# sun2ot/DiffMM

Hardware: NVIDIA B200
Metric: denoise_topk_rebuild_users_per_sec (higher is better)
Workload: dtype bf16

## Files before the change

diffmm_b200/csrc/adj.cu:

```cuda
#include "common.cuh"

#include <cub/device/device_radix_sort.cuh>

namespace {

__global__ void __launch_bounds__(256) expand_users_kernel(const int64_t* __restrict__ row_ptr, int64_t n_users,
                                                           int32_t* __restrict__ edge_user,
                                                           const int32_t* __restrict__ items, int64_t n_items,
                                                           int32_t* __restrict__ status) {
  const int64_t u = ((int64_t)blockIdx.x * blockDim.x + threadIdx.x) >> 5;
  const int lane = threadIdx.x & 31;
  if (u >= n_users) return;
  const int64_t b = row_ptr[u], e = row_ptr[u + 1];
  for (int64_t j = b + lane; j < e; j += 32) {
    edge_user[j] = (int32_t)u;
    const int32_t it = items[j];
    if ((it < 0 || it >= n_items) && status) atomicOr(status, 2);
  }
}

__device__ __forceinline__ int64_t lower_bound_item(const int32_t* __restrict__ items_sorted, int64_t n_edges, int64_t it) {
  int64_t lo = 0, hi = n_edges;
  while (lo < hi) {
    const int64_t mid = (lo + hi) >> 1;
    if ((int64_t)__ldg(items_sorted + mid) < it) lo = mid + 1; else hi = mid;
  }
  return lo;
}
__global__ void __launch_bounds__(256) offsets_dinv_kernel(const int64_t* __restrict__ row_ptr,
                                                           const int32_t* __restrict__ items_sorted, int64_t n_users,
                                                           int64_t n_items, int64_t n_edges, int64_t* __restrict__ item_ptr,
                                                           double* __restrict__ dinv) {
  __shared__ int64_t lb[256];
  const int64_t user_blocks = (n_users + 255) / 256;
  if ((int64_t)blockIdx.x < user_blocks) {
    const int64_t u = (int64_t)blockIdx.x * 256 + threadIdx.x;
    if (u < n_users) dinv[u] = 1.0 / sqrt((double)(row_ptr[u + 1] - row_ptr[u] + 1));
    return;
  }
  const int64_t it = ((int64_t)blockIdx.x - user_blocks) * 255 + threadIdx.x;
  lb[threadIdx.x] = it < n_items ? lower_bound_item(items_sorted, n_edges, it) : n_edges;
  __syncthreads();
  if (threadIdx.x == 255 || it >= n_items) return;
  const int64_t b = lb[threadIdx.x], e = lb[threadIdx.x + 1];
  item_ptr[it] = b;
  if (it + 1 == n_items) item_ptr[n_items] = n_edges;
  dinv[n_users + it] = 1.0 / sqrt((double)(e - b + 1));
}

__global__ void __launch_bounds__(256) fill_adj_kernel(const int64_t* __restrict__ row_ptr,
                                                       const int32_t* __restrict__ items,
                                                       const int32_t* __restrict__ edge_user,
                                                       const int64_t* __restrict__ item_ptr,
                                                       const int32_t* __restrict__ items_sorted,
                                                       const int32_t* __restrict__ users_by_item,
                                                       const double* __restrict__ dinv, int64_t n_users,
                                                       int64_t n_items, int64_t n_edges, int64_t* __restrict__ adj_ptr,
                                                       int32_t* __restrict__ adj_idx, float* __restrict__ adj_val) {
  const int64_t j = (int64_t)blockIdx.x * blockDim.x + threadIdx.x;
  const int64_t N = n_users + n_items;
  if (j < n_edges) {
    {
      const int64_t u = edge_user[j];
      const int32_t it = items[j];
      const int64_t o = j + u + 1;
      adj_idx[o] = (int32_t)(n_users + it);
      adj_val[o] = (float)((dinv[u] * 1.0) * dinv[n_users + it]);
    }
    {
      const int64_t it = items_sorted[j];
      const int32_t u = users_by_item[j];
      const int64_t o = n_edges + n_users + j + it;
      adj_idx[o] = u;
      adj_val[o] = (float)((dinv[n_users + it] * 1.0) * dinv[u]);
    }
  }
  if (j < N) {
    const double d = dinv[j];
    int64_t start, self;
    if (j < n_users) {
      start = row_ptr[j] + j;
      self = start;
    } else {
      const int64_t it = j - n_users;
      start = n_edges + n_users + item_ptr[it] + it;
      self = n_edges + n_users + item_ptr[it + 1] + it;
    }
    adj_ptr[j] = start;
    adj_idx[self] = (int32_t)j;
    adj_val[self] = (float)((d * 1.0) * d);
    if (j == N - 1) adj_ptr[N] = 2 * n_edges + N;
  }
}

struct Workspace {
  int32_t* edge_user;
  int32_t* items_sorted;
  int32_t* users_by_item;
  int32_t* item_count;
  int64_t* item_ptr;
  double* dinv;
  void* cub_tmp;
  size_t cub_bytes;
};

inline size_t align256(size_t x) { return (x + 255) & ~(size_t)255; }

inline size_t carve(Workspace& w, void* base, int64_t U, int64_t I, int64_t E) {
  uint8_t* p = (uint8_t*)base;
  size_t off = 0;
  const size_t e4 = align256((size_t)(E > 0 ? E : 1) * 4);
  w.edge_user = (int32_t*)(p + off); off += e4;
  w.items_sorted = (int32_t*)(p + off); off += e4;
  w.users_by_item = (int32_t*)(p + off); off += e4;
  w.item_count = (int32_t*)(p + off); off += align256((size_t)(I + 1) * 4);
  w.item_ptr = (int64_t*)(p + off); off += align256((size_t)(I + 1) * 8);
  w.dinv = (double*)(p + off); off += align256((size_t)(U + I) * 8);
  w.cub_tmp = p + off;
  return off;
}

}

extern "C" int64_t dmm_build_adj_workspace_bytes(int64_t n_users, int64_t n_items, int64_t n_edges) {
  Workspace w;
  const size_t fixed = carve(w, nullptr, n_users, n_items, n_edges);
  return (int64_t)(fixed + (size_t)(32u << 20) + (size_t)(n_edges > 0 ? n_edges : 0));
}

extern "C" int dmm_build_norm_adj_csr(dmm_ctx* ctx, const int64_t* row_ptr, const int32_t* items, int64_t n_users,
                                      int64_t n_items, int64_t n_edges, int64_t* adj_ptr, int32_t* adj_idx,
                                      float* adj_val, void* workspace, int64_t workspace_bytes, int32_t* status,
                                      void* stream) {
  DMM_CHECK_ARG(ctx && row_ptr && adj_ptr && adj_idx && adj_val && workspace, "dmm_build_norm_adj_csr: null argument");
  DMM_CHECK_ARG(n_users > 0 && n_items > 0 && n_edges >= 0, "dmm_build_norm_adj_csr: bad sizes");
  DMM_CHECK_ARG(n_users + n_items < (1LL << 31) && n_edges < (1LL << 31), "dmm_build_norm_adj_csr: int32 index overflow");
  DMM_CHECK_ARG(n_edges == 0 || items, "dmm_build_norm_adj_csr: null items");
  cudaStream_t st = (cudaStream_t)stream;
  Workspace w;
  const size_t fixed = carve(w, workspace, n_users, n_items, n_edges);
  DMM_CHECK_ARG((size_t)workspace_bytes > fixed, "dmm_build_norm_adj_csr: workspace too small");
  w.cub_bytes = (size_t)workspace_bytes - fixed;

  expand_users_kernel<<<(unsigned)dmm_ceil_div(n_users * 32, 256), 256, 0, st>>>(row_ptr, n_users, w.edge_user, items, n_items,
                                                                                status);
  DMM_LAUNCH_CHECK();
  if (n_edges > 0) {
    int end_bit = 1;
    while ((1LL << end_bit) < n_items) ++end_bit;
    size_t need = 0;
    DMM_CUDA(cub::DeviceRadixSort::SortPairs(nullptr, need, items, w.items_sorted, w.edge_user, w.users_by_item,
                                             (int)n_edges, 0, end_bit, st));
    if (need > w.cub_bytes) {
      dmm_set_error("dmm_build_norm_adj_csr: sort scratch needs %zu bytes, %zu available", need, w.cub_bytes);
      return DMM_ERR_WORKSPACE;
    }
    DMM_CUDA(cub::DeviceRadixSort::SortPairs(w.cub_tmp, need, items, w.items_sorted, w.edge_user, w.users_by_item,
                                             (int)n_edges, 0, end_bit, st));
  }
  const int64_t N = n_users + n_items;
  offsets_dinv_kernel<<<(unsigned)(dmm_ceil_div(n_users, 256) + dmm_ceil_div(n_items, 255)), 256, 0, st>>>(
      row_ptr, w.items_sorted, n_users, n_items, n_edges, w.item_ptr, w.dinv);
  DMM_LAUNCH_CHECK();
  const int64_t work = n_edges > N ? n_edges : N;
  fill_adj_kernel<<<(unsigned)dmm_ceil_div(work, 256), 256, 0, st>>>(row_ptr, items, w.edge_user, w.item_ptr, w.items_sorted,
                                                                    w.users_by_item, w.dinv, n_users, n_items, n_edges,
                                                                    adj_ptr, adj_idx, adj_val);
  DMM_LAUNCH_CHECK();
  return DMM_OK;
}
```

diffmm_b200/csrc/topk.cu:

```cuda
#include "common.cuh"

#include <stdlib.h>

namespace {

constexpr int TOPK_NB_LOG2 = 11;
constexpr int TOPK_NB = 1 << TOPK_NB_LOG2;
constexpr int TOPK_CAND = 1024;
constexpr int TOPK_V4 = 8;
constexpr int TOPK_SEG_COLS = 8192;
constexpr int TOPK_MERGE_CAP = 2048;

struct SegCfg {
  int mode;
  int S;
  int seg_cols;
  int last_len;
};
__device__ __forceinline__ bool seg_eligible(const SegCfg& sg, int k) {
  return k > 0 && k <= 256 && k <= sg.last_len && (int64_t)sg.S * k <= TOPK_MERGE_CAP;
}

__device__ __forceinline__ float fmax_nan(float a, float b) {
  float r;
// ... 403 lines not shown
      const float xs[4] = {v[j].x, v[j].y, v[j].z, v[j].w};
#pragma unroll
      for (int e = 0; e < 4; ++e) push(open && !(xs[e] < Lf), xs[e], 4 * (tid + NT * j) + e);
    }
  }
  if (n_cols & 3) push(has_tail && !(tail_v < Lf), tail_v, tail_col);
  __syncthreads();
  const int m = sm.ncand;
  constexpr int RANK_MAX = 512;
  if (m > RANK_MAX || m < k) {
    __syncthreads();
    topk_row_generic<NT, false>(sm, nullptr, row, n_cols, k, o0, user, out_users, out_items, col_off);
    return;
  }
  for (int c = tid; c < m; c += NT) {
    const uint32_t my_key = sm.cand[c];
    const int my_col = sm.cand_col[c];
    int before = 0;
    if (m > k) {
      for (int j = 0; j < m; ++j) {
        const uint32_t kj = sm.cand[j];
        const int cj = sm.cand_col[j];
        before += (kj > my_key || (kj == my_key && cj < my_col)) ? 1 : 0;
      }
    }
    sm.bucket[c] = before < k ? my_col : 0x7FFFFFFF;
  }
  __syncthreads();
  for (int c = tid; c < m; c += NT) {
    const int my_col = sm.bucket[c];
    if (my_col == 0x7FFFFFFF) continue;
    int pos = 0;
    for (int j = 0; j < m; ++j) pos += (sm.bucket[j] < my_col) ? 1 : 0;
    out_items[o0 + pos] = my_col + col_off;
    if (out_users) out_users[o0 + pos] = user;
  }
}

__global__ void __launch_bounds__(128) topk_merge_kernel(const float* __restrict__ scores, int64_t ld, int64_t n_rows,
                                                         const int64_t* __restrict__ out_ptr, int64_t row_base,
                                                         int32_t* __restrict__ out_users, int32_t* __restrict__ out_items,
                                                         const int32_t* __restrict__ order, SegCfg sg,
                                                         const int32_t* __restrict__ seg_tmp, const int32_t* __restrict__ live) {
  __shared__ uint32_t key[TOPK_MERGE_CAP];
  __shared__ int col[TOPK_MERGE_CAP];
  __shared__ int sel[TOPK_MERGE_CAP];
  if ((int64_t)blockIdx.x >= n_rows) return;
  if (live && (int64_t)blockIdx.x >= (int64_t)*live) return;
  const int64_t r = order ? (int64_t)order[blockIdx.x] : (int64_t)blockIdx.x;
  const int64_t o0 = out_ptr[r];
  const int k = (int)(out_ptr[r + 1] - o0);
  if (!seg_eligible(sg, k)) return;
  const int m = sg.S * k;
  const int32_t* list = seg_tmp + (int64_t)sg.S * (o0 - out_ptr[0]);
  const float* row = scores + r * ld;
  for (int c = threadIdx.x; c < m; c += 128) {
    const int cc = list[c];
    col[c] = cc;
    key[c] = order_key(__ldg(row + cc));
  }
  __syncthreads();
  for (int c = threadIdx.x; c < m; c += 128) {
    const uint32_t my_key = key[c];
    const int my_col = col[c];
    int before = 0;
    for (int j = 0; j < m; ++j) before += (key[j] > my_key || (key[j] == my_key && col[j] < my_col)) ? 1 : 0;
    sel[c] = before < k ? my_col : 0x7FFFFFFF;
  }
  __syncthreads();
  const int32_t user = (int32_t)(row_base + r);
  for (int c = threadIdx.x; c < m; c += 128) {
    const int my_col = sel[c];
    if (my_col == 0x7FFFFFFF) continue;
    int pos = 0;
    for (int j = 0; j < m; ++j) pos += (sel[j] < my_col) ? 1 : 0;
    out_items[o0 + pos] = my_col;
    if (out_users) out_users[o0 + pos] = user;
  }
}

template <int NT>
void launch_reg(const float* scores, int64_t ld, int64_t n_rows, int n_cols, const int64_t* out_ptr, int64_t row_base,
                int32_t* out_users, int32_t* out_items, int32_t* status, const int32_t* order, SegCfg sg, int32_t* seg_tmp,
                const int32_t* live, cudaStream_t st) {
  const int64_t blocks = sg.mode == 1 ? n_rows * sg.S : n_rows;
  topk_rows_reg_kernel<NT><<<(unsigned)blocks, NT, 0, st>>>(scores, ld, n_rows, n_cols, out_ptr, row_base, out_users,
                                                           out_items, status, order, sg, seg_tmp, live);
}

constexpr int PRUNE_KMAX = 64;
constexpr int PRUNE_RATIO = 4;
constexpr int PRUNE_CAND = 512;

struct PruneArgs {
  const float* scores;
  int64_t ld;
  const float* cmax;
  int64_t ld_cmax;
  int n_chunks, n_cols;
  int64_t n_rows;
  const int64_t* out_ptr;
  int64_t row_base;
  int32_t* out_users;
  int32_t* out_items;
  int32_t* status;
  const int32_t* order;
  int32_t* left_count;
  int32_t* left_rows;
};

__host__ __device__ __forceinline__ int prune_kmax(int n_chunks) {
  const int nw = n_chunks <= 64 * 4 * TOPK_V4 ? 2 : (n_chunks <= 256 * 4 * TOPK_V4 ? 8 : 16);
  return PRUNE_KMAX < 32 * nw ? PRUNE_KMAX : 32 * nw;
}
__host__ __device__ __forceinline__ bool prune_k_ok(int64_t k, int n_chunks, int64_t n_cols) {
  return k <= prune_kmax(n_chunks) && k * PRUNE_RATIO <= n_chunks && k <= n_cols;
}

struct alignas(16) PruneSmem {
  uint32_t key[PRUNE_CAND];
  int col[PRUNE_CAND];
  int sel[PRUNE_CAND];
  uint32_t red[32];
  int ncand, nsel, ncand2;
  uint32_t lk;
};

__device__ __forceinline__ float key_to_float(uint32_t L) {
  return (L == 0u) ? __uint_as_float(0xFF800000u) : __uint_as_float((L & 0x80000000u) ? (L ^ 0x80000000u) : ~L);
}

template <int NT>
__global__ void __launch_bounds__(NT) topk_pruned_kernel(const PruneArgs a) {
  __shared__ PruneSmem sm;
  constexpr int NW = NT / 32;
  if ((int64_t)blockIdx.x >= a.n_rows) return;
  const int64_t r = a.order ? (int64_t)a.order[blockIdx.x] : (int64_t)blockIdx.x;
  const int tid = threadIdx.x, lane = tid & 31, wid = tid >> 5;
  const int n_chunks = a.n_chunks;

  const float* crow = a.cmax + r * a.ld_cmax;
  const int n4 = n_chunks >> 2;
  const float4* crow4 = reinterpret_cast<const float4*>(crow);
  float4 v[TOPK_V4];
#pragma unroll
  for (int j = 0; j < TOPK_V4; ++j) {
    v[j] = make_float4(0.f, 0.f, 0.f, 0.f);
    if (tid + NT * j < n4) v[j] = __ldg(crow4 + tid + NT * j);
  }
  const int tail_col = (n4 << 2) + tid;
  const bool has_tail = tid < (n_chunks & 3);
  float tail_v = 0.f;
  if (has_tail) tail_v = __ldg(crow + tail_col);

  const int64_t o0 = a.out_ptr[r];
  const int k = (int)(a.out_ptr[r + 1] - o0);
  if (k <= 0) return;
  auto defer = [&]() {
    if (tid == 0) a.left_rows[atomicAdd(a.left_count, 1)] = (int32_t)r;
  };
  if (!prune_k_ok(k, n_chunks, a.n_cols)) {
    defer();
    return;
  }
  const float NEG_INF = __uint_as_float(0xFF800000u);
  const int jfull = n4 / NT, jrem = n4 - jfull * NT;
  float pmax[TOPK_V4];
  float tmaxf = has_tail ? fmax_nan(tail_v, NEG_INF) : NEG_INF;
#pragma unroll
  for (int j = 0; j < TOPK_V4; ++j) {
    pmax[j] = NEG_INF;
    if (j < jfull || (j == jfull && tid < jrem)) {
      pmax[j] = fmax_nan(fmax_nan(v[j].x, v[j].y), fmax_nan(v[j].z, v[j].w));
      tmaxf = fmax_nan(tmaxf, pmax[j]);
    }
  }
  const uint32_t tmax = (tmaxf == NEG_INF) ? 0u : order_key(tmaxf);

  const int q = (k + NW - 1) / NW;
  uint32_t wq;
  {
    uint32_t sv = tmax;
#pragma unroll
    for (int k2 = 2; k2 <= 32; k2 <<= 1) {
#pragma unroll
      for (int j = k2 >> 1; j > 0; j >>= 1) {
        const uint32_t other = __shfl_xor_sync(0xffffffffu, sv, j);
        const bool desc = (lane & k2) == 0;
        const bool lower = (lane & j) == 0;
        sv = (lower == desc) ? max(sv, other) : min(sv, other);
      }
    }
    wq = __shfl_sync(0xffffffffu, sv, q - 1);
  }
  if (lane == 0) sm.red[wid] = wq;
  if (tid == 0) {
    sm.ncand = 0;
    sm.nsel = 0;
    sm.ncand2 = 0;
    sm.lk = 0xFFFFFFFFu;
  }
  if (__syncthreads_or(tmaxf != tmaxf)) {
    defer();
    return;
  }
  uint32_t L = 0xFFFFFFFFu;
#pragma unroll
  for (int i = 0; i < NW; ++i) L = min(L, sm.red[i]);
  const float Lf = key_to_float(L);

  auto push = [&](int* counter, bool c, float x, int col) {
    const uint32_t bal = __ballot_sync(0xffffffffu, c);
    if (bal) {
      int base = 0;
      if (lane == 0) base = atomicAdd(counter, __popc(bal));
      base = __shfl_sync(0xffffffffu, base, 0);
      const int pos = base + __popc(bal & ((1u << lane) - 1u));
      if (c && pos < PRUNE_CAND) {
        sm.key[pos] = order_key(x);
        sm.col[pos] = col;
      }
    }
  };
#pragma unroll
  for (int j = 0; j < TOPK_V4; ++j) {
    if (j > jfull) break;
    const bool have = j < jfull || tid < jrem;
    const bool open = have && !(pmax[j] < Lf);
    if (__any_sync(0xffffffffu, open)) {
      const float xs[4] = {v[j].x, v[j].y, v[j].z, v[j].w};
#pragma unroll
      for (int e = 0; e < 4; ++e) push(&sm.ncand, open && !(xs[e] < Lf), xs[e], 4 * (tid + NT * j) + e);
    }
  }
  if (n_chunks & 3) push(&sm.ncand, has_tail && !(tail_v < Lf), tail_v, tail_col);
  __syncthreads();
  const int m = sm.ncand;
  if (m > PRUNE_CAND || m < k) {
    defer();
    return;
  }
  for (int c = tid; c < m; c += NT) {
    const uint32_t my_key = sm.key[c];
    const int my_col = sm.col[c];
    int before = 0;
    if (m > k) {
      for (int j = 0; j < m; ++j) {
        const uint32_t kj = sm.key[j];
        const int cj = sm.col[j];
        before += (kj > my_key || (kj == my_key && cj < my_col)) ? 1 : 0;
      }
    }
    if (before < k) {
      sm.sel[atomicAdd(&sm.nsel, 1)] = my_col;
      atomicMin(&sm.lk, my_key);
    }
  }
  __syncthreads();
  const float Lkf = key_to_float(sm.lk);

  const float* row = a.scores + r * a.ld;
  constexpr int GB = 8;
  for (int i0 = wid; i0 < k; i0 += NW * GB) {
    float xs[GB];
    int cols[GB];
#pragma unroll
    for (int t = 0; t < GB; ++t) {
      const int i = i0 + t * NW;
      cols[t] = i < k ? sm.sel[i] * 32 + lane : 0x7FFFFFFF;
      xs[t] = cols[t] < a.n_cols ? __ldg(row + cols[t]) : NEG_INF;
    }
#pragma unroll
    for (int t = 0; t < GB; ++t) {
      if (i0 + t * NW >= k) break;
      push(&sm.ncand2, cols[t] < a.n_cols && !(xs[t] < Lkf), xs[t], cols[t]);
    }
  }
  __syncthreads();
  const int m2 = sm.ncand2;
  if (m2 > PRUNE_CAND || m2 < k) {
    defer();
    return;
  }
  for (int c = tid; c < m2; c += NT) {
    const uint32_t my_key = sm.key[c];
    const int my_col = sm.col[c];
    int before = 0;
    if (m2 > k) {
      for (int j = 0; j < m2; ++j) {
        const uint32_t kj = sm.key[j];
        const int cj = sm.col[j];
        before += (kj > my_key || (kj == my_key && cj < my_col)) ? 1 : 0;
      }
    }
    sm.sel[c] = before < k ? my_col : 0x7FFFFFFF;
  }
  __syncthreads();
  const int32_t user = (int32_t)(a.row_base + r);
  for (int c = tid; c < m2; c += NT) {
    const int my_col = sm.sel[c];
    if (my_col == 0x7FFFFFFF) continue;
    int pos = 0;
    for (int j = 0; j < m2; ++j) pos += (sm.sel[j] < my_col) ? 1 : 0;
    a.out_items[o0 + pos] = my_col;
    if (a.out_users) a.out_users[o0 + pos] = user;
  }
}

__global__ void __launch_bounds__(256) topk_deferred_kernel(const float* __restrict__ scores, int64_t ld, int n_cols,
                                                            const float* __restrict__ cmax, int64_t ld_cmax, int n_chunks,
                                                            const int64_t* __restrict__ out_ptr, int64_t row_base,
                                                            int32_t* __restrict__ out_users, int32_t* __restrict__ out_items,
                                                            int32_t* __restrict__ status, const int32_t* __restrict__ rows,
                                                            const int32_t* __restrict__ live,
                                                            int32_t* __restrict__ chunk_list, int smem_keys) {
  extern __shared__ uint32_t s_keys[];
  __shared__ TopkSmem<256> sm;
  const int tid = threadIdx.x;
  const int n = *live;
  const int64_t e0 = out_ptr[0];
  for (int slot = blockIdx.x; slot < n; slot += gridDim.x) {
    const int64_t r = rows[slot];
    const int64_t o0 = out_ptr[r];
    int k = (int)(out_ptr[r + 1] - o0);
    if (k > n_cols) {
      if (status && tid == 0) atomicOr(status, 1);
      k = n_cols;
    }
    if (k <= 0) continue;
    const float* row = scores + r * ld;
    const float* crow = cmax + r * ld_cmax;
    bool two_level = (int64_t)k * 2 <= n_chunks;
    if (two_level) {
      bool nan = false;
      for (int i = tid; i < n_chunks; i += 256) {
        const float c = __ldg(crow + i);
        nan |= c != c;
      }
      two_level = !__syncthreads_or(nan);
    }
    if (two_level) {
      int32_t* list = chunk_list + (o0 - e0);
      if (n_chunks <= smem_keys) {
        uint32_t kmin = 0xFFFFFFFFu, kmax = 0u;
        for (int i = tid; i < n_chunks; i += 256) {
          const uint32_t q = order_key(__ldg(crow + i));
          s_keys[i] = q;
          kmin = min(kmin, q);
          kmax = max(kmax, q);
        }
        topk_select_emit<256>(sm, [&](int i) -> uint32_t { return s_keys[i]; }, [](int i) -> int { return i; }, n_chunks, k,
                              true, kmin, kmax, 0, 0, nullptr, list);
      } else {
        topk_select_emit<256>(sm, [&](int i) -> uint32_t { return order_key(__ldg(crow + i)); }, [](int i) -> int { return i; },
                              n_chunks, k, false, 0u, 0u, 0, 0, nullptr, list);
      }
      __syncthreads();
      const int nv = k * 32;
      auto vcol = [&](int i) -> int { return list[i >> 5] * 32 + (i & 31); };
      auto vkey = [&](int i) -> uint32_t {
        const int c = vcol(i);
        return c < n_cols ? order_key(__ldg(row + c)) : 0u;
      };
      if (nv <= smem_keys) {
        uint32_t kmin = 0xFFFFFFFFu, kmax = 0u;
#pragma unroll 4
        for (int i = tid; i < nv; i += 256) {
          const uint32_t q = vkey(i);
          s_keys[i] = q;
          kmin = min(kmin, q);
          kmax = max(kmax, q);
        }
        topk_select_emit<256>(sm, [&](int i) -> uint32_t { return s_keys[i]; }, vcol, nv, k, true, kmin, kmax, o0,
                              (int32_t)(row_base + r), out_users, out_items);
      } else {
        topk_select_emit<256>(sm, vkey, vcol, nv, k, false, 0u, 0u, o0, (int32_t)(row_base + r), out_users, out_items);
      }
    } else {
      topk_row_generic<256, false>(sm, nullptr, row, n_cols, k, o0, (int32_t)(row_base + r), out_users, out_items);
    }
    __syncthreads();
  }
}

SegCfg make_seg(int64_t n_cols) {
  SegCfg sg{0, 0, 0, 0};
  if (n_cols > TOPK_SEG_COLS) {
    sg.S = (int)dmm_ceil_div(n_cols, TOPK_SEG_COLS);
    sg.seg_cols = (int)((dmm_ceil_div(n_cols, sg.S) + 3) / 4 * 4);
    sg.last_len = (int)(n_cols - (int64_t)(sg.S - 1) * sg.seg_cols);
    if (sg.last_len <= 0) sg.S = 0;
  }
  return sg;
}

}

extern "C" int64_t dmm_topk_workspace_bytes(int64_t n_cols, int64_t n_edges) {
  const SegCfg sg = make_seg(n_cols);
  return sg.S > 0 ? (int64_t)sg.S * (n_edges > 0 ? n_edges : 0) * (int64_t)sizeof(int32_t) : 0;
}

static int topk_dispatch(dmm_ctx* ctx, const float* scores, int64_t ld, int64_t n_rows, int64_t n_cols,
                         const int64_t* out_ptr, int64_t row_base, int32_t* out_users, int32_t* out_items, int32_t* status,
                         const int32_t* order, const int32_t* live, void* workspace, int64_t workspace_bytes,
                         int64_t n_edges, cudaStream_t st) {
  constexpr int PER_THREAD = 4 * TOPK_V4;
  static const bool force_generic = getenv("DMM_TOPK_GENERIC") != nullptr;
  static const bool seg_ok = []() { const char* e = getenv("DMM_TOPK_SEG"); return !(e && e[0] == '0'); }();

  SegCfg sg = make_seg(n_cols);
  const bool rows_aligned = (reinterpret_cast<uintptr_t>(scores) & 15u) == 0 && ld % 4 == 0;
  const bool segmented = seg_ok && !force_generic && sg.S > 0 && rows_aligned && workspace != nullptr && n_edges >= 0 &&
                         workspace_bytes >= dmm_topk_workspace_bytes(n_cols, n_edges) && n_rows * (int64_t)sg.S < (1LL << 31);
  if (segmented) {
    sg.mode = 1;
    launch_reg<256>(scores, ld, n_rows, (int)n_cols, out_ptr, row_base, nullptr, nullptr, status, order, sg, (int32_t*)workspace,
                    live, st);
    DMM_LAUNCH_CHECK();
    topk_merge_kernel<<<(unsigned)n_rows, 128, 0, st>>>(scores, ld, n_rows, out_ptr, row_base, out_users, out_items, order, sg,
                                                       (const int32_t*)workspace, live);
    DMM_LAUNCH_CHECK();
    sg.mode = 2;
    topk_edges_kernel<false><<<(unsigned)n_rows, 256, 0, st>>>(scores, ld, n_rows, (int)n_cols, out_ptr, row_base, out_users,
                                                              out_items, status, order, sg, live);
    DMM_LAUNCH_CHECK();
    return DMM_OK;
  }
  sg = SegCfg{0, 0, 0, 0};
  if (force_generic) {
  } else if (n_cols <= 256 * PER_THREAD) {
    launch_reg<256>(scores, ld, n_rows, (int)n_cols, out_ptr, row_base, out_users, out_items, status, order, sg, nullptr, live, st);
  } else if (n_cols <= 512 * PER_THREAD) {
    launch_reg<512>(scores, ld, n_rows, (int)n_cols, out_ptr, row_base, out_users, out_items, status, order, sg, nullptr, live, st);
  } else if (n_cols <= 1024 * PER_THREAD) {
    launch_reg<1024>(scores, ld, n_rows, (int)n_cols, out_ptr, row_base, out_users, out_items, status, order, sg, nullptr, live, st);
  }
  if (force_generic || n_cols > 1024 * PER_THREAD) {
    const size_t smem = (size_t)n_cols * sizeof(uint32_t);
    const size_t cap = (size_t)ctx->max_smem_optin > 40960 ? (size_t)ctx->max_smem_optin - 20480 : 0;
    if (smem <= cap) {
      static DmmPerDeviceOnce smem_once;
      if (smem > 24 * 1024 && smem_once.need(ctx)) {
        DMM_CUDA(cudaFuncSetAttribute(topk_edges_kernel<true>, cudaFuncAttributeMaxDynamicSharedMemorySize, (int)cap));
        smem_once.mark(ctx);
      }
      topk_edges_kernel<true><<<(unsigned)n_rows, 256, smem, st>>>(scores, ld, n_rows, (int)n_cols, out_ptr, row_base,
                                                                  out_users, out_items, status, order, sg, live);
    } else {
      topk_edges_kernel<false><<<(unsigned)n_rows, 256, 0, st>>>(scores, ld, n_rows, (int)n_cols, out_ptr, row_base,
                                                                out_users, out_items, status, order, sg, live);
    }
  }
  DMM_LAUNCH_CHECK();
  return DMM_OK;
}

extern "C" int dmm_topk_edges(dmm_ctx* ctx, const float* scores, int64_t ld, int64_t n_rows, int64_t n_cols,
                              const int64_t* out_ptr, int64_t row_base, int32_t* out_users, int32_t* out_items,
                              int32_t* status, const int32_t* order, void* workspace, int64_t workspace_bytes,
                              int64_t n_edges, void* stream) {
  DMM_CHECK_ARG(ctx && scores && out_ptr && out_items, "dmm_topk_edges: null argument");
  DMM_CHECK_ARG(n_cols > 0 && n_cols < (1LL << 31) && ld >= n_cols, "dmm_topk_edges: bad shape n_cols=%lld ld=%lld",
                (long long)n_cols, (long long)ld);
  DMM_CHECK_ARG(n_rows >= 0 && n_rows < (1LL << 31), "dmm_topk_edges: bad n_rows");
  if (n_rows == 0) return DMM_OK;
  return topk_dispatch(ctx, scores, ld, n_rows, n_cols, out_ptr, row_base, out_users, out_items, status, order, nullptr,
                       workspace, workspace_bytes, n_edges, (cudaStream_t)stream);
}

namespace {
inline size_t prune_align(size_t x) { return (x + 255) & ~(size_t)255; }
inline size_t prune_head_bytes(int64_t n_rows) { return 256 + prune_align((size_t)(n_rows > 0 ? n_rows : 1) * sizeof(int32_t)); }
}

extern "C" int64_t dmm_topk_pruned_workspace_bytes(int64_t n_rows, int64_t n_cols, int64_t n_edges) {
  return (int64_t)prune_head_bytes(n_rows) + (int64_t)prune_align((size_t)(n_edges > 0 ? n_edges : 1) * sizeof(int32_t)) +
         dmm_topk_workspace_bytes(n_cols, n_edges);
}

extern "C" int dmm_topk_edges_pruned(dmm_ctx* ctx, const float* scores, int64_t ld, int64_t n_rows, int64_t n_cols,
                                     const float* cmax, int64_t ld_cmax, const int64_t* out_ptr, int64_t row_base,
                                     int32_t* out_users, int32_t* out_items, int32_t* status, const int32_t* order,
                                     void* workspace, int64_t workspace_bytes, int64_t n_edges, void* stream) {
  DMM_CHECK_ARG(ctx && scores && cmax && out_ptr && out_items && workspace, "dmm_topk_edges_pruned: null argument");
  DMM_CHECK_ARG(n_cols > 0 && n_cols < (1LL << 31) && ld >= n_cols, "dmm_topk_edges_pruned: bad shape n_cols=%lld ld=%lld",
                (long long)n_cols, (long long)ld);
  DMM_CHECK_ARG(n_rows >= 0 && n_rows < (1LL << 31) && n_edges >= 0, "dmm_topk_edges_pruned: bad n_rows / n_edges");
  const int64_t n_chunks = dmm_ceil_div(n_cols, 32);
  DMM_CHECK_ARG(ld_cmax >= n_chunks && ld_cmax % 4 == 0 && (reinterpret_cast<uintptr_t>(cmax) & 15u) == 0,
                "dmm_topk_edges_pruned: cmax rows must be 16-byte aligned with ld_cmax %% 4 == 0 and >= ceil(n_cols / 32)");
  DMM_CHECK_ARG(workspace_bytes >= dmm_topk_pruned_workspace_bytes(n_rows, n_cols, n_edges),
                "dmm_topk_edges_pruned: workspace smaller than dmm_topk_pruned_workspace_bytes");
  if (n_rows == 0) return DMM_OK;
  cudaStream_t st = (cudaStream_t)stream;
  const size_t list_bytes = prune_align((size_t)(n_edges > 0 ? n_edges : 1) * sizeof(int32_t));
  int32_t* const chunk_list = (int32_t*)((uint8_t*)workspace + prune_head_bytes(n_rows));
  uint8_t* const seg_ws = (uint8_t*)workspace + prune_head_bytes(n_rows) + list_bytes;
  const int64_t seg_ws_bytes = workspace_bytes - (int64_t)prune_head_bytes(n_rows) - (int64_t)list_bytes;
  static const bool prune_ok = []() { const char* e = getenv("DMM_TOPK_PRUNE"); return !(e && e[0] == '0'); }();
  if (!prune_ok || n_chunks > 512 * 4 * TOPK_V4 || n_chunks < 8)
    return topk_dispatch(ctx, scores, ld, n_rows, n_cols, out_ptr, row_base, out_users, out_items, status, order, nullptr,
                         seg_ws, seg_ws_bytes, n_edges, st);
  int32_t* left_count = (int32_t*)workspace;
  int32_t* left_rows = (int32_t*)((uint8_t*)workspace + 256);
  DMM_CUDA(cudaMemsetAsync(left_count, 0, sizeof(int32_t), st));
  const PruneArgs a{scores, ld, cmax, ld_cmax, (int)n_chunks, (int)n_cols, n_rows, out_ptr, row_base, out_users, out_items,
                    status, order, left_count, left_rows};
  if (n_chunks <= 64 * 4 * TOPK_V4) topk_pruned_kernel<64><<<(unsigned)n_rows, 64, 0, st>>>(a);
  else if (n_chunks <= 256 * 4 * TOPK_V4) topk_pruned_kernel<256><<<(unsigned)n_rows, 256, 0, st>>>(a);
  else topk_pruned_kernel<512><<<(unsigned)n_rows, 512, 0, st>>>(a);
  DMM_LAUNCH_CHECK();
  constexpr int SMEM_KEYS = 20480;
  static DmmPerDeviceOnce attr_once;
  if (attr_once.need(ctx)) {
    DMM_CUDA(cudaFuncSetAttribute(topk_deferred_kernel, cudaFuncAttributeMaxDynamicSharedMemorySize, SMEM_KEYS * 4));
    attr_once.mark(ctx);
  }
  topk_deferred_kernel<<<(unsigned)(ctx->num_sms * 2), 256, SMEM_KEYS * 4, st>>>(
      scores, ld, (int)n_cols, cmax, ld_cmax, (int)n_chunks, out_ptr, row_base, out_users, out_items, status, left_rows,
      left_count, chunk_list, SMEM_KEYS);
  DMM_LAUNCH_CHECK();
  return DMM_OK;
}
```

Baseline: 14.59 million.

## Replace radix sort with tiled counting sort for adjacency and add warp-per-row pruned top-k

When there are few items, the normalized adjacency build replaces the CUB radix sort by item with a three-kernel counting sort. Each tile counts items in packed 16-bit shared-memory histograms, the per-tile counts are scanned per item, and a scatter kernel ranks edges using warp match-any. Separately, rows with small chunk counts in pruned top-k are handled one warp per row, four rows per block, instead of one CTA per row, which cuts block overhead and the block-wide syncs. The changes add code paths gated on size thresholds, and the counting sort relies on a last-block-done pattern to finish the scan.

```diff
diff --git a/diffmm_b200/csrc/adj.cu b/diffmm_b200/csrc/adj.cu
--- a/diffmm_b200/csrc/adj.cu
+++ b/diffmm_b200/csrc/adj.cu
@@ -3,6 +3,232 @@
 #include <cub/device/device_radix_sort.cuh>
 
 namespace {
+
+constexpr int CS_NT = 256;
+constexpr int64_t CS_TILE_MIN = 1024;
+constexpr int64_t CS_TILE_MAX = 8192;
+constexpr int64_t CS_COUNT_CAP = 1 << 21;
+constexpr int64_t CS_ITEMS_MAX = 65536;
+
+struct CsPlan {
+  bool on;
+  int64_t tiles, tile;
+};
+
+inline CsPlan cs_plan(int64_t n_items, int64_t n_edges) {
+  CsPlan p{false, 1, 32};
+  if (n_items > CS_ITEMS_MAX) return p;
+  if (n_edges > 0) {
+    int64_t t = dmm_ceil_div(n_edges, CS_TILE_MIN);
+    const int64_t cap = CS_COUNT_CAP / n_items;
+    if (t > cap) t = cap;
+    if (t < 1) t = 1;
+    p.tile = dmm_ceil_div(dmm_ceil_div(n_edges, t), 32) * 32;
+    p.tiles = dmm_ceil_div(n_edges, p.tile);
+  }
+  p.on = p.tile <= CS_TILE_MAX;
+  return p;
+}
+
+inline size_t cs_scatter_smem(int64_t n_items, int64_t tile) {
+  return (size_t)((n_items + 1) >> 1) * 4 + (size_t)tile * 4 + (size_t)tile * 2;
+}
+constexpr int CS_COUNT_SMEM_MAX = (int)(CS_ITEMS_MAX / 2 * 4);
+constexpr int CS_SCATTER_SMEM_MAX = (int)(CS_ITEMS_MAX / 2 * 4 + CS_TILE_MAX * 6);
+static_assert(CS_SCATTER_SMEM_MAX <= 200 * 1024, "the scatter kernel's shared memory must fit an sm_100 CTA");
+
+__device__ __forceinline__ int32_t clamp_item(int32_t it, int64_t n_items, bool& bad) {
+  if (it < 0 || it >= n_items) {
+    bad = true;
+    return it < 0 ? 0 : (int32_t)(n_items - 1);
+  }
+  return it;
+}
+
+__device__ __forceinline__ int64_t user_of_edge(const int64_t* __restrict__ row_ptr, int64_t n_users, int64_t j) {
+  int64_t lo = 0, hi = n_users;
+  while (hi - lo > 1) {
+    const int64_t mid = (lo + hi) >> 1;
+    if (row_ptr[mid] <= j) lo = mid; else hi = mid;
+  }
+  return lo;
+}
+
+__global__ void __launch_bounds__(CS_NT) cs_count_kernel(const int64_t* __restrict__ row_ptr, int64_t n_users,
+                                                         const int32_t* __restrict__ items, int64_t n_items,
+                                                         int64_t n_edges, int64_t tile, int32_t* __restrict__ edge_user,
+                                                         int32_t* __restrict__ counts, int32_t* __restrict__ status,
+                                                         int32_t* __restrict__ done) {
+  extern __shared__ uint32_t s_cnt[];
+  __shared__ int64_t s_u[2];
+  const int tid = threadIdx.x, lane = tid & 31, warp = tid >> 5;
+  const int64_t words = (n_items + 1) >> 1;
+  for (int64_t i = tid; i < words; i += CS_NT) s_cnt[i] = 0u;
+  if (blockIdx.x == 0 && tid == 0) *done = 0;
+  const int64_t j0 = (int64_t)blockIdx.x * tile;
+  const int64_t j1 = min(j0 + tile, n_edges);
+  if (tid < 2 && j0 < j1) s_u[tid] = user_of_edge(row_ptr, n_users, tid == 0 ? j0 : j1 - 1);
+  __syncthreads();
+  bool bad = false;
+  for (int64_t j = j0 + tid; j < j1; j += CS_NT) {
+    const int32_t it = clamp_item(items[j], n_items, bad);
+    atomicAdd(&s_cnt[it >> 1], 1u << ((it & 1) * 16));
+  }
+  if (bad && status) atomicOr(status, 2);
+  if (j0 < j1) {
+    for (int64_t u = s_u[0] + warp; u <= s_u[1]; u += CS_NT / 32) {
+      const int64_t b = max(row_ptr[u], j0), e = min(row_ptr[u + 1], j1);
+      for (int64_t j = b + lane; j < e; j += 32) edge_user[j] = (int32_t)u;
+    }
+  }
+  __syncthreads();
+  int32_t* row = counts + (int64_t)blockIdx.x * n_items;
+  for (int64_t it = tid; it < n_items; it += CS_NT) row[it] = (int32_t)((s_cnt[it >> 1] >> ((it & 1) * 16)) & 0xFFFFu);
+}
+
+__global__ void __launch_bounds__(CS_NT) cs_scan_kernel(const int64_t* __restrict__ row_ptr, int64_t n_users,
+                                                        int64_t n_items, int64_t n_edges, int64_t tiles,
+                                                        int32_t* __restrict__ counts, int32_t* __restrict__ item_deg,
+                                                        int64_t* __restrict__ item_ptr, double* __restrict__ dinv,
+                                                        int32_t* __restrict__ done) {
+  constexpr int G = CS_NT / 32;
+  constexpr int B = 8;
+  __shared__ int s_sum[G][32];
+  __shared__ int64_t s_scan[CS_NT / 32];
+  __shared__ bool s_last;
+  const int tid = threadIdx.x, lane = tid & 31, g = tid >> 5;
+  const int64_t it = (int64_t)blockIdx.x * 32 + lane;
+  const int64_t per = (tiles + G - 1) / G;
+  const int64_t t0 = min((int64_t)g * per, tiles), t1 = min(t0 + per, tiles);
+  int32_t* col = counts + it;
+  int sum = 0;
+  if (it < n_items) {
+#pragma unroll B
+    for (int64_t t = t0; t < t1; ++t) sum += col[t * n_items];
+  }
+  s_sum[g][lane] = sum;
+  __syncthreads();
+  int run = 0, tot = 0;
+#pragma unroll
+  for (int h = 0; h < G; ++h) {
+    const int s = s_sum[h][lane];
+    if (h < g) run += s;
+    tot += s;
+  }
+  if (it < n_items) {
+    for (int64_t t = t0; t < t1; t += B) {
+      int c[B];
+#pragma unroll
+      for (int b = 0; b < B; ++b) c[b] = t + b < t1 ? col[(t + b) * n_items] : 0;
+#pragma unroll
+      for (int b = 0; b < B; ++b) {
+        if (t + b < t1) col[(t + b) * n_items] = run;
+        run += c[b];
+      }
+    }
+    if (g == 0) item_deg[it] = tot;
+  }
+  for (int64_t u = (int64_t)blockIdx.x * CS_NT + tid; u < n_users; u += (int64_t)gridDim.x * CS_NT)
+    dinv[u] = 1.0 / sqrt((double)(row_ptr[u + 1] - row_ptr[u] + 1));
+
+  __threadfence();
+  __syncthreads();
+  if (tid == 0) s_last = atomicAdd(done, 1) == (int)gridDim.x - 1;
+  __syncthreads();
+  if (!s_last) return;
+  __threadfence();
+  const int64_t run_len = (n_items + CS_NT - 1) / CS_NT;
+  const int64_t b0 = min((int64_t)tid * run_len, n_items), b1 = min(b0 + run_len, n_items);
+  int64_t part = 0;
+  for (int64_t i = b0; i < b1; ++i) part += __ldcg(item_deg + i);
+  int64_t incl = part;
+#pragma unroll
+  for (int o = 1; o < 32; o <<= 1) {
+    const int64_t y = __shfl_up_sync(0xffffffffu, incl, o);
+    if (lane >= o) incl += y;
+  }
+  if (lane == 31) s_scan[g] = incl;
+  __syncthreads();
+  int64_t base = incl - part;
+  for (int h = 0; h < g; ++h) base += s_scan[h];
+  for (int64_t i = b0; i < b1; ++i) {
+    const int d = __ldcg(item_deg + i);
+    item_ptr[i] = base;
+    dinv[n_users + i] = 1.0 / sqrt((double)(d + 1));
+    base += d;
+  }
+  if (tid == 0) item_ptr[n_items] = n_edges;
+}
+
+__global__ void __launch_bounds__(CS_NT) cs_scatter_kernel(const int64_t* __restrict__ row_ptr,
+                                                           const int32_t* __restrict__ items,
+                                                           const int32_t* __restrict__ edge_user,
+                                                           const int32_t* __restrict__ counts,
+                                                           const int64_t* __restrict__ item_ptr,
+                                                           const double* __restrict__ dinv, int64_t n_users,
+                                                           int64_t n_items, int64_t n_edges, int64_t tile,
+                                                           int64_t* __restrict__ adj_ptr, int32_t* __restrict__ adj_idx,
+                                                           float* __restrict__ adj_val) {
+  extern __shared__ uint32_t smem[];
+  const int64_t words = (n_items + 1) >> 1;
+  uint32_t* s_cur = smem;
+  int32_t* s_item = reinterpret_cast<int32_t*>(smem + words);
+  uint16_t* s_rank = reinterpret_cast<uint16_t*>(s_item + tile);
+  const int tid = threadIdx.x, lane = tid & 31;
+  const int64_t j0 = (int64_t)blockIdx.x * tile;
+  const int n = (int)max((int64_t)0, min(tile, n_edges - j0));
+  for (int64_t i = tid; i < words; i += CS_NT) s_cur[i] = 0u;
+  for (int e = tid; e < n; e += CS_NT) s_item[e] = min(max(items[j0 + e], 0), (int32_t)(n_items - 1));
+  __syncthreads();
+  const int64_t N = n_users + n_items;
+  if (tid < 32) {
+    for (int e0 = 0; e0 < n; e0 += 32) {
+      const int e = e0 + lane;
+      const bool valid = e < n;
+      const int32_t it = valid ? s_item[e] : -1;
+      const uint32_t peers = __match_any_sync(0xffffffffu, it);
+      const int leader = __ffs(peers) - 1;
+      const int sh = (it & 1) * 16;
+      uint32_t old = 0u;
+      if (valid && lane == leader) old = atomicAdd(&s_cur[it >> 1], (uint32_t)__popc(peers) << sh);
+      old = __shfl_sync(0xffffffffu, old, leader);
+      if (valid) s_rank[e] = (uint16_t)(((old >> sh) & 0xFFFFu) + __popc(peers & ((1u << lane) - 1u)));
+    }
+  } else {
+    constexpr int NO = CS_NT - 32;
+    for (int64_t v = (int64_t)blockIdx.x * NO + (tid - 32); v < N; v += (int64_t)gridDim.x * NO) {
+      const double d = dinv[v];
+      int64_t start, self;
+      if (v < n_users) {
+        start = row_ptr[v] + v;
+        self = start;
+      } else {
+        const int64_t it = v - n_users;
+        start = n_edges + n_users + item_ptr[it] + it;
+        self = n_edges + n_users + item_ptr[it + 1] + it;
+      }
+      adj_ptr[v] = start;
+      adj_idx[self] = (int32_t)v;
+      adj_val[self] = (float)((d * 1.0) * d);
+      if (v == N - 1) adj_ptr[N] = 2 * n_edges + N;
+    }
+  }
+  __syncthreads();
+  const int32_t* base = counts + (int64_t)blockIdx.x * n_items;
+  for (int e = tid; e < n; e += CS_NT) {
+    const int64_t j = j0 + e;
+    const int64_t u = edge_user[j];
+    const int32_t it = s_item[e];
+    const double du = dinv[u], di = dinv[n_users + it];
+    const int64_t o = j + u + 1;
+    adj_idx[o] = (int32_t)(n_users + it);
+    adj_val[o] = (float)((du * 1.0) * di);
+    const int64_t pos = item_ptr[it] + base[it] + s_rank[e];
+    const int64_t o2 = n_edges + n_users + pos + it;
+    adj_idx[o2] = (int32_t)u;
+    adj_val[o2] = (float)((di * 1.0) * du);
+  }
+}
 
 __global__ void __launch_bounds__(256) expand_users_kernel(const int64_t* __restrict__ row_ptr, int64_t n_users,
                                                            int32_t* __restrict__ edge_user,
@@ -95,27 +321,33 @@
 
 struct Workspace {
   int32_t* edge_user;
+  int32_t* item_deg;
+  int64_t* item_ptr;
+  double* dinv;
+  int32_t* counts;
   int32_t* items_sorted;
   int32_t* users_by_item;
-  int32_t* item_count;
-  int64_t* item_ptr;
-  double* dinv;
   void* cub_tmp;
   size_t cub_bytes;
 };
 
 inline size_t align256(size_t x) { return (x + 255) & ~(size_t)255; }
 
-inline size_t carve(Workspace& w, void* base, int64_t U, int64_t I, int64_t E) {
+inline size_t carve(Workspace& w, void* base, int64_t U, int64_t I, int64_t E, const CsPlan& cs) {
   uint8_t* p = (uint8_t*)base;
   size_t off = 0;
   const size_t e4 = align256((size_t)(E > 0 ? E : 1) * 4);
   w.edge_user = (int32_t*)(p + off); off += e4;
-  w.items_sorted = (int32_t*)(p + off); off += e4;
-  w.users_by_item = (int32_t*)(p + off); off += e4;
-  w.item_count = (int32_t*)(p + off); off += align256((size_t)(I + 1) * 4);
+  w.item_deg = (int32_t*)(p + off); off += align256((size_t)(I + 1) * 4);
   w.item_ptr = (int64_t*)(p + off); off += align256((size_t)(I + 1) * 8);
   w.dinv = (double*)(p + off); off += align256((size_t)(U + I) * 8);
+  w.counts = w.items_sorted = w.users_by_item = nullptr;
+  if (cs.on) {
+    w.counts = (int32_t*)(p + off); off += align256((size_t)(cs.tiles * I) * 4);
+  } else {
+    w.items_sorted = (int32_t*)(p + off); off += e4;
+    w.users_by_item = (int32_t*)(p + off); off += e4;
+  }
   w.cub_tmp = p + off;
   return off;
 }
@@ -124,7 +356,9 @@
 
 extern "C" int64_t dmm_build_adj_workspace_bytes(int64_t n_users, int64_t n_items, int64_t n_edges) {
   Workspace w;
-  const size_t fixed = carve(w, nullptr, n_users, n_items, n_edges);
+  const CsPlan cs = cs_plan(n_items, n_edges);
+  const size_t fixed = carve(w, nullptr, n_users, n_items, n_edges, cs);
+  if (cs.on) return (int64_t)fixed;
   return (int64_t)(fixed + (size_t)(32u << 20) + (size_t)(n_edges > 0 ? n_edges : 0));
 }
 
@@ -137,10 +371,35 @@
   DMM_CHECK_ARG(n_users + n_items < (1LL << 31) && n_edges < (1LL << 31), "dmm_build_norm_adj_csr: int32 index overflow");
   DMM_CHECK_ARG(n_edges == 0 || items, "dmm_build_norm_adj_csr: null items");
   cudaStream_t st = (cudaStream_t)stream;
+  const CsPlan cs = cs_plan(n_items, n_edges);
   Workspace w;
-  const size_t fixed = carve(w, workspace, n_users, n_items, n_edges);
-  DMM_CHECK_ARG((size_t)workspace_bytes > fixed, "dmm_build_norm_adj_csr: workspace too small");
+  const size_t fixed = carve(w, workspace, n_users, n_items, n_edges, cs);
+  DMM_CHECK_ARG((size_t)workspace_bytes >= fixed, "dmm_build_norm_adj_csr: workspace too small");
   w.cub_bytes = (size_t)workspace_bytes - fixed;
+  const int64_t N = n_users + n_items;
+
+  if (cs.on) {
+    const size_t count_smem = (size_t)((n_items + 1) >> 1) * 4;
+    const size_t scatter_smem = cs_scatter_smem(n_items, cs.tile);
+    static DmmPerDeviceOnce attr_once;
+    if (attr_once.need(ctx)) {
+      DMM_CUDA(cudaFuncSetAttribute(cs_count_kernel, cudaFuncAttributeMaxDynamicSharedMemorySize, CS_COUNT_SMEM_MAX));
+      DMM_CUDA(cudaFuncSetAttribute(cs_scatter_kernel, cudaFuncAttributeMaxDynamicSharedMemorySize, CS_SCATTER_SMEM_MAX));
+      attr_once.mark(ctx);
+    }
+    int32_t* done = w.item_deg + n_items;
+    cs_count_kernel<<<(unsigned)cs.tiles, CS_NT, count_smem, st>>>(row_ptr, n_users, items, n_items, n_edges, cs.tile,
+                                                                    w.edge_user, w.counts, status, done);
+    DMM_LAUNCH_CHECK();
+    cs_scan_kernel<<<(unsigned)dmm_ceil_div(n_items, 32), CS_NT, 0, st>>>(row_ptr, n_users, n_items, n_edges, cs.tiles,
+                                                                          w.counts, w.item_deg, w.item_ptr, w.dinv, done);
+    DMM_LAUNCH_CHECK();
+    cs_scatter_kernel<<<(unsigned)cs.tiles, CS_NT, scatter_smem, st>>>(row_ptr, items, w.edge_user, w.counts, w.item_ptr,
+                                                                       w.dinv, n_users, n_items, n_edges, cs.tile, adj_ptr,
+                                                                       adj_idx, adj_val);
+    DMM_LAUNCH_CHECK();
+    return DMM_OK;
+  }
 
   expand_users_kernel<<<(unsigned)dmm_ceil_div(n_users * 32, 256), 256, 0, st>>>(row_ptr, n_users, w.edge_user, items, n_items,
                                                                                 status);
@@ -158,7 +417,6 @@
     DMM_CUDA(cub::DeviceRadixSort::SortPairs(w.cub_tmp, need, items, w.items_sorted, w.edge_user, w.users_by_item,
                                              (int)n_edges, 0, end_bit, st));
   }
-  const int64_t N = n_users + n_items;
   offsets_dinv_kernel<<<(unsigned)(dmm_ceil_div(n_users, 256) + dmm_ceil_div(n_items, 255)), 256, 0, st>>>(
       row_ptr, w.items_sorted, n_users, n_items, n_edges, w.item_ptr, w.dinv);
   DMM_LAUNCH_CHECK();
diff --git a/diffmm_b200/csrc/topk.cu b/diffmm_b200/csrc/topk.cu
--- a/diffmm_b200/csrc/topk.cu
+++ b/diffmm_b200/csrc/topk.cu
@@ -729,6 +729,167 @@
     if (my_col == 0x7FFFFFFF) continue;
     int pos = 0;
     for (int j = 0; j < m2; ++j) pos += (sm.sel[j] < my_col) ? 1 : 0;
+    a.out_items[o0 + pos] = my_col;
+    if (a.out_users) a.out_users[o0 + pos] = user;
+  }
+}
+
+constexpr int PW_WARPS = 4;
+constexpr int PW_KMAX = 32;
+constexpr int PW_CAND = 128;
+
+__global__ void __launch_bounds__(32 * PW_WARPS) topk_pruned_warp_kernel(const PruneArgs a) {
+  __shared__ uint32_t s_key[PW_WARPS][PW_CAND];
+  __shared__ int s_col[PW_WARPS][PW_CAND];
+  __shared__ int s_sel[PW_WARPS][PW_CAND];
+  const int lane = threadIdx.x & 31, wid = threadIdx.x >> 5;
+  const int64_t slot = (int64_t)blockIdx.x * PW_WARPS + wid;
+  if (slot >= a.n_rows) return;
+  const int64_t r = a.order ? (int64_t)a.order[slot] : slot;
+  uint32_t* key = s_key[wid];
+  int* col = s_col[wid];
+  int* sel = s_sel[wid];
+  const int n_chunks = a.n_chunks;
+  const unsigned FULL = 0xffffffffu;
+
+  const float* crow = a.cmax + r * a.ld_cmax;
+  const int n4 = n_chunks >> 2;
+  const float4* crow4 = reinterpret_cast<const float4*>(crow);
+  float4 v[TOPK_V4];
+#pragma unroll
+  for (int j = 0; j < TOPK_V4; ++j) {
+    v[j] = make_float4(0.f, 0.f, 0.f, 0.f);
+    if (lane + 32 * j < n4) v[j] = __ldg(crow4 + lane + 32 * j);
+  }
+  const int tail_col = (n4 << 2) + lane;
+  const bool has_tail = lane < (n_chunks & 3);
+  float tail_v = 0.f;
+  if (has_tail) tail_v = __ldg(crow + tail_col);
+
+  const int64_t o0 = a.out_ptr[r];
+  const int k = (int)(a.out_ptr[r + 1] - o0);
+  if (k <= 0) return;
+  auto defer = [&]() {
+    if (lane == 0) a.left_rows[atomicAdd(a.left_count, 1)] = (int32_t)r;
+  };
+  if (!(k <= PW_KMAX && k * PRUNE_RATIO <= n_chunks && k <= a.n_cols)) {
+    defer();
+    return;
+  }
+  const float NEG_INF = __uint_as_float(0xFF800000u);
+  const int jfull = n4 / 32, jrem = n4 - jfull * 32;
+  float pmax[TOPK_V4];
+  float tmaxf = has_tail ? fmax_nan(tail_v, NEG_INF) : NEG_INF;
+#pragma unroll
+  for (int j = 0; j < TOPK_V4; ++j) {
+    pmax[j] = NEG_INF;
+    if (j < jfull || (j == jfull && lane < jrem)) {
+      pmax[j] = fmax_nan(fmax_nan(v[j].x, v[j].y), fmax_nan(v[j].z, v[j].w));
+      tmaxf = fmax_nan(tmaxf, pmax[j]);
+    }
+  }
+  if (__any_sync(FULL, tmaxf != tmaxf)) {
+    defer();
+    return;
+  }
+  uint32_t sv = (tmaxf == NEG_INF) ? 0u : order_key(tmaxf);
+#pragma unroll
+  for (int k2 = 2; k2 <= 32; k2 <<= 1) {
+#pragma unroll
+    for (int j = k2 >> 1; j > 0; j >>= 1) {
+      const uint32_t other = __shfl_xor_sync(FULL, sv, j);
+      const bool desc = (lane & k2) == 0;
+      const bool lower = (lane & j) == 0;
+      sv = (lower == desc) ? max(sv, other) : min(sv, other);
+    }
+  }
+  const float Lf = key_to_float(__shfl_sync(FULL, sv, k - 1));
+
+  const uint32_t lt = (1u << lane) - 1u;
+  int m = 0;
+  auto push = [&](bool c, float x, int cc) {
+    const uint32_t bal = __ballot_sync(FULL, c);
+    const int pos = m + __popc(bal & lt);
+    if (c && pos < PW_CAND) {
+      key[pos] = order_key(x);
+      col[pos] = cc;
+    }
+    m += __popc(bal);
+  };
+#pragma unroll
+  for (int j = 0; j < TOPK_V4; ++j) {
+    if (j > jfull) break;
+    const bool have = j < jfull || lane < jrem;
+    const bool open = have && !(pmax[j] < Lf);
+    if (__any_sync(FULL, open)) {
+      const float xs[4] = {v[j].x, v[j].y, v[j].z, v[j].w};
+#pragma unroll
+      for (int e = 0; e < 4; ++e) push(open && !(xs[e] < Lf), xs[e], 4 * (lane + 32 * j) + e);
+    }
+  }
+  if (n_chunks & 3) push(has_tail && !(tail_v < Lf), tail_v, tail_col);
+  __syncwarp();
+  if (m > PW_CAND || m < k) {
+    defer();
+    return;
+  }
+  uint32_t lk = 0xFFFFFFFFu;
+  for (int c = lane; c < m; c += 32) {
+    const uint32_t my_key = key[c];
+    const int my_col = col[c];
+    int before = 0;
+    for (int j = 0; j < m; ++j) {
+      const uint32_t kj = key[j];
+      before += (kj > my_key || (kj == my_key && col[j] < my_col)) ? 1 : 0;
+    }
+    if (before < k) {
+      sel[before] = my_col;
+      lk = min(lk, my_key);
+    }
+  }
+  const float Lkf = key_to_float(__reduce_min_sync(FULL, lk));
+  __syncwarp();
+
+  const float* row = a.scores + r * a.ld;
+  float xs[PW_KMAX];
+  int cs[PW_KMAX];
+#pragma unroll
+  for (int t = 0; t < PW_KMAX; ++t) {
+    cs[t] = t < k ? sel[t] * 32 + lane : 0x7FFFFFFF;
+    xs[t] = cs[t] < a.n_cols ? __ldg(row + cs[t]) : NEG_INF;
+  }
+  __syncwarp();
+  m = 0;
+#pragma unroll
+  for (int t = 0; t < PW_KMAX; ++t) {
+    if (t >= k) break;
+    push(cs[t] < a.n_cols && !(xs[t] < Lkf), xs[t], cs[t]);
+  }
+  __syncwarp();
+  const int m2 = m;
+  if (m2 > PW_CAND || m2 < k) {
+    defer();
+    return;
+  }
+  for (int c = lane; c < m2; c += 32) {
+    const uint32_t my_key = key[c];
+    const int my_col = col[c];
+    int before = 0;
+    if (m2 > k) {
+      for (int j = 0; j < m2; ++j) {
+        const uint32_t kj = key[j];
+        before += (kj > my_key || (kj == my_key && col[j] < my_col)) ? 1 : 0;
+      }
+    }
+    sel[c] = before < k ? my_col : 0x7FFFFFFF;
+  }
+  __syncwarp();
+  const int32_t user = (int32_t)(a.row_base + r);
+  for (int c = lane; c < m2; c += 32) {
+    const int my_col = sel[c];
+    if (my_col == 0x7FFFFFFF) continue;
+    int pos = 0;
+    for (int j = 0; j < m2; ++j) pos += (sel[j] < my_col) ? 1 : 0;
     a.out_items[o0 + pos] = my_col;
     if (a.out_users) a.out_users[o0 + pos] = user;
   }
@@ -934,7 +1095,9 @@
   DMM_CUDA(cudaMemsetAsync(left_count, 0, sizeof(int32_t), st));
   const PruneArgs a{scores, ld, cmax, ld_cmax, (int)n_chunks, (int)n_cols, n_rows, out_ptr, row_base, out_users, out_items,
                     status, order, left_count, left_rows};
-  if (n_chunks <= 64 * 4 * TOPK_V4) topk_pruned_kernel<64><<<(unsigned)n_rows, 64, 0, st>>>(a);
+  if (n_chunks <= 32 * 4 * TOPK_V4)
+    topk_pruned_warp_kernel<<<(unsigned)dmm_ceil_div(n_rows, PW_WARPS), 32 * PW_WARPS, 0, st>>>(a);
+  else if (n_chunks <= 64 * 4 * TOPK_V4) topk_pruned_kernel<64><<<(unsigned)n_rows, 64, 0, st>>>(a);
   else if (n_chunks <= 256 * 4 * TOPK_V4) topk_pruned_kernel<256><<<(unsigned)n_rows, 256, 0, st>>>(a);
   else topk_pruned_kernel<512><<<(unsigned)n_rows, 512, 0, st>>>(a);
   DMM_LAUNCH_CHECK();
```

Result: slower. 14.19 million (median of 6 runs) (-2.7%).
